# retrojetpacks/Gadget-Leicester

Measured on AMD Instinct MI355X. Metric: particle-steps/sec (gravity+SPH), higher is better.
Workload: dtype f64

## Files before the change

gadget-leicester_amd/csrc/ghip_gravity.hip:

```cpp
#include <cmath>

#include "ghip_prim.h"
#include "ghip_walk.h"

__global__ void k_grav_finish(int nt, const int *__restrict__ tgt, const int *__restrict__ perm,
                              int n, double G, double comoving_fac, const double *__restrict__ pos,
                              const double *__restrict__ gravpm, double *__restrict__ oacc,
                              double *__restrict__ oldacc)
{
  int ti = blockIdx.x * blockDim.x + threadIdx.x;
  if(ti >= nt)
    return;
  int i = perm[tgt[ti]];
  double a0 = oacc[i], a1 = oacc[(size_t) n + i], a2 = oacc[2 * (size_t) n + i];
  if(comoving_fac != 0)
    {
      a0 += comoving_fac * pos[i];
      a1 += comoving_fac * pos[(size_t) n + i];
      a2 += comoving_fac * pos[2 * (size_t) n + i];
    }
  double b0 = a0, b1 = a1, b2 = a2;
  if(gravpm)
    {
      b0 = a0 + gravpm[i] / G;
// ... 333 lines not shown
    sg.nsub = 1;
  sg.start = P<int>(t.seg_start) + t.seg_soff[table];
  sg.nanc = P<int>(t.seg_nanc) + t.seg_noff[table];
  sg.anc = P<int>(t.seg_anc) + (size_t) t.seg_noff[table] * GHIP_MAXANC;
  return sg.nsub;
}

static int walk_layout(const TreeDev &t, int nt, WalkSeg &sg, int *nbuckets, bool ewald)
{
  *nbuckets = (nt + 63) / 64;
  static int mid_min = -1;
  if(mid_min < 0)
    {
      mid_min = 3072;
      if(getenv("GHIP_WALK_MID_MIN"))
        mid_min = atoi(getenv("GHIP_WALK_MID_MIN"));
    }
  int table = ewald ? (*nbuckets >= mid_min ? 2 : 1) : (*nbuckets >= mid_min ? 1 : 0);
  return ghip_walk_layout(t, sg, table);
}

struct PartialBufs
{
  double *ax, *ay, *az;
  int *cost;
};

static int ensure_partials(ghip_ctx *ctx, int nwaves, int slot, PartialBufs &pb)
{
  size_t cnt = (size_t) nwaves * 64;
  DevBuf &bx = slot ? ctx->tax2 : ctx->tax, &by = slot ? ctx->tay2 : ctx->tay,
         &bz = slot ? ctx->taz2 : ctx->taz, &bc = slot ? ctx->tcost2 : ctx->tcost;
  GCHK(ghip_ensure(ctx, bx, cnt * 8));
  GCHK(ghip_ensure(ctx, by, cnt * 8));
  GCHK(ghip_ensure(ctx, bz, cnt * 8));
  GCHK(ghip_ensure(ctx, bc, cnt * 4));
  pb.ax = P<double>(bx);
  pb.ay = P<double>(by);
  pb.az = P<double>(bz);
  pb.cost = P<int>(bc);
  return GHIP_OK;
}

static int build_plan(ghip_ctx *ctx, int kind, int nb, int ns, WalkPlan &plan, int slot = 0,
                      hipStream_t on = nullptr)
{
  hipStream_t st = on ? on : ctx->stream;
  DevBuf &b_nsub = slot ? ctx->plan_nsub2 : ctx->plan_nsub, &b_woff = slot ? ctx->plan_woff2 : ctx->plan_woff,
         &b_wave = slot ? ctx->plan_wave2 : ctx->plan_wave;
  int sbase = (49152 + nb - 1) / nb;
  sbase = sbase < 8 ? 8 : (sbase > 64 ? 64 : sbase);
  if(sbase > ns)
    sbase = ns;
  if(getenv("GHIP_WALK_SUBS"))
    {
      int v = atoi(getenv("GHIP_WALK_SUBS"));
      if(v >= 1 && v <= ns)
        sbase = v;
    }
  const int maxwaves = (sbase + 2) * nb + 8;
  GCHK(ghip_ensure(ctx, b_nsub, (size_t) nb * 4));
  GCHK(ghip_ensure(ctx, b_woff, (size_t) (nb + 1) * 4));
  GCHK(ghip_ensure(ctx, b_wave, (size_t) maxwaves * 4));
  int cur = ctx->plan_cur[kind];
  bool prev_kept = ctx->plan_steps[kind][cur].p != nullptr;
  const size_t steps_bytes = ((size_t) nb + nb / 8 + 64) * 4;
  for(int k = 0; k < 2; k++)
    if(ctx->plan_steps[kind][k].cap < (size_t) nb * 4)
      {
        GCHK(ghip_ensure(ctx, ctx->plan_steps[kind][k], steps_bytes));
        if(k == cur)
          prev_kept = false;
      }
  const bool adaptive = !(getenv("GHIP_WALK_ADAPTIVE") && atoi(getenv("GHIP_WALK_ADAPTIVE")) == 0);
  const int pnb = ctx->plan_nb[kind];
  int tol = nb / 16 < 8 ? 8 : nb / 16;
  if(getenv("GHIP_PLAN_EXACT") && atoi(getenv("GHIP_PLAN_EXACT")))
    tol = ctx->plan_ns[kind] == ns ? 0 : -1;
  bool have_prev = adaptive && kind < 2 && pnb > 0 && (pnb > nb ? pnb - nb : nb - pnb) <= tol && prev_kept;
  int nprev = have_prev ? (pnb < nb ? pnb : nb) : 0;
  if(getenv("GHIP_PLAN_DEBUG") && kind < 2)
    {
      static int calls[2], used[2];
      calls[kind]++;
      used[kind] += have_prev;
      if(calls[kind] % 16 == 0)
        fprintf(stderr, "ghip plan kind %d: history used in %d of %d calls (nb %d, before %d)\n", kind,
                used[kind], calls[kind], nb, pnb);
    }
  unsigned int *prev = P<unsigned int>(ctx->plan_steps[kind][cur]);
  unsigned int *out = P<unsigned int>(ctx->plan_steps[kind][cur ^ 1]);
  k_plan_nsub<<<cdiv(nb, 256), 256, 0, st>>>(nb, ns, sbase, prev, nprev, P<int>(b_nsub));
  GCHK(ghip_scan(ctx, P<int>(b_nsub), P<int>(b_woff), nb, st, slot ? &ghip_prim_scratch(ctx, ctx->stream2) : nullptr));
  HIPCHK(hipMemsetAsync(b_wave.p, 0xff, (size_t) maxwaves * 4, st));
  k_plan_fill<<<cdiv(nb, 256), 256, 0, st>>>(nb, P<int>(b_nsub), P<int>(b_woff),
                                             maxwaves, P<int>(b_wave), out,
                                             ghip_errword(ctx, GHIP_ERRW_PLAN));
  HIPCHK(hipGetLastError());
  if(kind < 2)
    {
      ctx->plan_nb[kind] = nb;
      ctx->plan_ns[kind] = ns;
      ctx->plan_cur[kind] = cur ^ 1;
    }
  plan.nwaves = maxwaves;
  plan.wave_bucket = P<int>(b_wave);
  plan.woff = P<int>(b_woff);
  plan.nsub = P<int>(b_nsub);
  plan.steps_out = out;
  plan.started = nullptr;
  plan.started_at = 0;
  return GHIP_OK;
}

template <int MODE>
static void launch_walk(ghip_ctx *ctx, const TreeDev &t, const WalkSeg &sg, int nbuckets, int nt,
                        const int *tgt, const double *tx, const double *ty, const double *tz,
                        const double *tsoft, const double *toldacc, const GravK &k,
                        unsigned long long *counter, const WalkPlan &plan, const PartialBufs &pb,
                        hipStream_t stream)
{
  long long nthreads = (long long) plan.nwaves * 64;
  int bsize = 64;
  if(getenv("GHIP_WALK_BLOCK"))
    {
      int v = atoi(getenv("GHIP_WALK_BLOCK"));
      if(v == 64 || v == 128 || v == 256)
        bsize = v;
    }
  int blocks = cdiv(nthreads, bsize);
  blocks = (blocks + 7) & ~7;
  if(k.xcd_remap > 1)
    blocks = ((blocks + 8 * k.xcd_remap - 1) / (8 * k.xcd_remap)) * (8 * k.xcd_remap);
  WalkPlan pl = plan;
  if(pl.started)
    {
      static double frac = -1;
      if(frac < 0)
        frac = getenv("GHIP_HYDRO_TRIGGER_AT") ? atof(getenv("GHIP_HYDRO_TRIGGER_AT")) : 1.0;
      pl.started_at = (int) (frac * (blocks - 1));
      if(pl.started_at > blocks - 1 || pl.started_at < 0)
        pl.started_at = blocks - 1;
    }
  static int lds_env = -1;
  if(lds_env < 0)
    lds_env = getenv("GHIP_PAIR_NEWTON_LDS") ? atoi(getenv("GHIP_PAIR_NEWTON_LDS")) : 0;
  const int lds_n = lds_env > 0 ? lds_env : ctx->pair_lds;
  static int cap_min = -1;
  if(cap_min < 0)
    cap_min = getenv("GHIP_PAIR_CAP_MIN") ? atoi(getenv("GHIP_PAIR_CAP_MIN")) : 1536;
  static int lds_e = -1;
  if(lds_e < 0)
    lds_e = getenv("GHIP_PAIR_EWALD_LDS") ? atoi(getenv("GHIP_PAIR_EWALD_LDS")) : 0;
  const size_t dyn_lds =
    (MODE == GHIP_WALK_NEWTON && stream != ctx->stream && nbuckets >= cap_min)
      ? (size_t) lds_n
      : ((MODE == GHIP_WALK_EWALD && stream != ctx->stream && nbuckets >= cap_min) ? (size_t) lds_e : 0);
#define GHIP_LAUNCH_WALK(PER, UNEQ)                                                              \
  k_grav_walk<MODE, PER, UNEQ><<<blocks, bsize, dyn_lds, stream>>>(                                \
    t.nelem, P<WalkHot>(t.mq), P<WalkCold>(t.mq2), sg, nt, tgt, tx, ty, tz, tsoft, toldacc, k,     \
    P<float>(ctx->srtab), P<double>((UNEQ) && MODE == GHIP_WALK_EWALD ? ctx->ewbrick : ctx->ewtab),  \
    pb.ax, pb.ay, pb.az, pb.cost, getenv("GHIP_WALK_NOCOUNT") ? nullptr : counter,                  \
    P<unsigned long long>(ctx->rslots) + (counter - P<unsigned long long>(ctx->cslots)), pl)
  static int brick_env = -2;
  if(brick_env == -2)
    brick_env = getenv("GHIP_EW_BRICK") ? atoi(getenv("GHIP_EW_BRICK")) : -1;
  const bool brick = brick_env >= 0 ? brick_env != 0 : true;
  const bool uneq = (MODE == GHIP_WALK_EWALD) ? brick : (bool) k.unequal;
  if(k.periodic && uneq)
    GHIP_LAUNCH_WALK(true, true);
  else if(k.periodic)
    GHIP_LAUNCH_WALK(true, false);
  else if(uneq)
    GHIP_LAUNCH_WALK(false, true);
  else
    GHIP_LAUNCH_WALK(false, false);
#undef GHIP_LAUNCH_WALK
}

static void launch_walk_any(ghip_ctx *ctx, int walk, const TreeDev &t, const WalkSeg &sg,
                            int nbuckets, int nt, const int *tgt, const double *tx,
                            const double *ty, const double *tz, const double *tsoft,
                            const double *toldacc, const GravK &k, unsigned long long *counter,
                            const WalkPlan &plan, const PartialBufs &pb, hipStream_t stream)
{
  if(walk == GHIP_WALK_NEWTON)
    launch_walk<GHIP_WALK_NEWTON>(ctx, t, sg, nbuckets, nt, tgt, tx, ty, tz, tsoft, toldacc, k,
                                  counter, plan, pb, stream);
  else if(walk == GHIP_WALK_SHORTRANGE)
    launch_walk<GHIP_WALK_SHORTRANGE>(ctx, t, sg, nbuckets, nt, tgt, tx, ty, tz, tsoft, toldacc, k,
                                      counter, plan, pb, stream);
  else
    launch_walk<GHIP_WALK_EWALD>(ctx, t, sg, nbuckets, nt, tgt, tx, ty, tz, tsoft, toldacc, k,
                                 counter, plan, pb, stream);
}

static void shard_slice(const ghip_ctx *ctx, int nt, int *lo, int *cnt)
{
  int per;
  ghip_shard_range(nt, ctx->shard_n, ctx->shard_rank, lo, cnt, &per);
}

struct WalkJob
{
  int walk;
  GravK k;
  WalkSeg sg;
  WalkPlan plan;
  PartialBufs pb;
  int nbuckets;
  unsigned long long *counter;
};

static int prepare_job(ghip_ctx *ctx, const ghip_grav_params *p, int walk, int nt, int slot,
                       WalkJob &J, hipStream_t plan_on = nullptr)
{
  hipStream_t ps = plan_on ? plan_on : ctx->stream;
  J.walk = walk;
  GCHK(prepare_tables(ctx, p, walk, J.k));
  walk_layout(ctx->dyn_use ? ctx->dyn.tree : ctx->gt, nt, J.sg, &J.nbuckets, walk == GHIP_WALK_EWALD);
  GCHK(build_plan(ctx, walk == GHIP_WALK_EWALD ? 1 : 0, J.nbuckets, J.sg.ns, J.plan, slot, ps));
  GCHK(ensure_partials(ctx, J.plan.nwaves, slot, J.pb));
  J.counter = ghip_cslot(ctx, walk == GHIP_WALK_EWALD ? GHIP_CK_EWALD : GHIP_CK_NEWTON);
  HIPCHK(hipMemsetAsync(J.counter, 0, GHIP_CKIND_U64 * 8, ps));
  return GHIP_OK;
}

static int run_walk(ghip_ctx *ctx, const WalkJob &J, int nt, const int *tgt, hipStream_t st)
{
  int evi = (J.walk == GHIP_WALK_EWALD) ? 4 : 2;
  ctx->plan_writer[J.walk == GHIP_WALK_EWALD ? 1 : 0] = st;
  HIPCHK(hipEventRecord(ctx->evp[evi], st));
  launch_walk_any(ctx, J.walk, ctx->dyn_use ? ctx->dyn.tree : ctx->gt, J.sg, J.nbuckets, nt, tgt, P<double>(ctx->sx),
                  P<double>(ctx->sy), P<double>(ctx->sz), P<double>(ctx->ssoft),
                  P<double>(ctx->soldacc), J.k, J.counter, J.plan, J.pb, st);
  HIPCHK(hipGetLastError());
  HIPCHK(hipEventRecord(ctx->evp[evi + 1], st));
  return GHIP_OK;
}

static int combine_walk(ghip_ctx *ctx, const WalkJob &J, int nt, const int *tgt, hipStream_t st)
{
  k_combine_grav<<<cdiv(nt, 256), 256, 0, st>>>(
    nt, J.plan, tgt, P<int>(ctx->gt.perm), J.pb.ax, J.pb.ay, J.pb.az, J.pb.cost, ctx->n,
    P<double>(ctx->f[GHIP_F_GRAVACCEL]), P<int>(ctx->f[GHIP_F_GRAVCOST]),
    J.walk == GHIP_WALK_EWALD ? 1 : 0, J.k.debug_steps);
  HIPCHK(hipGetLastError());
  return GHIP_OK;
}

static const int pair_caps[GHIP_PAIR_NSET] = {GHIP_PAIR_LDS(6), GHIP_PAIR_LDS(5), GHIP_PAIR_LDS(4)};

static int pair_setting(int lds)
{
  int k = 0;
  for(int j = 1; j < GHIP_PAIR_NSET; j++)
    if(lds >= pair_caps[j])
      k = j;
  return k;
}

static int pair_balance(ghip_ctx *ctx)
{
  if(!ctx->pc_ev[3][3])
    {
      for(int i = 0; i < 4; i++)
        for(int j = 0; j < 4; j++)
          if(!ctx->pc_ev[i][j])
            HIPCHK(hipEventCreate(&ctx->pc_ev[i][j]));
      return GHIP_OK;
    }
  bool pending[GHIP_PAIR_NSET] = {};
  for(int i = 0; i < 4; i++)
    {
      if(ctx->pc_cap[i] == 0)
        continue;
      hipEvent_t *e = ctx->pc_ev[i];
      if(hipEventQuery(e[1]) != hipSuccess || hipEventQuery(e[3]) != hipSuccess)
        {
          (void) hipGetLastError();
          pending[pair_setting(ctx->pc_cap[i])] = true;
          continue;
        }
      float tn = 0, te = 0;
      if(hipEventElapsedTime(&tn, e[0], e[1]) == hipSuccess && hipEventElapsedTime(&te, e[2], e[3]) == hipSuccess)
        {
          const int k = pair_setting(ctx->pc_cap[i]);
          const float fe = ctx->pc_hyd[i] ? 1.1f : 1.0f;
          const float c = tn > fe * te ? tn : fe * te;
          ctx->pc_cost[k] = c;
          ctx->pc_age[k] = 0;
        }
      else
        (void) hipGetLastError();
      ctx->pc_cap[i] = 0;
    }
  for(int k = 0; k < GHIP_PAIR_NSET; k++)
    ctx->pc_age[k]++;
  const int cur = pair_setting(ctx->pair_lds);
  const float *cost = ctx->pc_cost;
  if(cost[cur] < 0)
    return GHIP_OK;
  int want = cur, probe = -1;
  for(int k = 0; k < GHIP_PAIR_NSET; k++)
    {
      if(k == cur || pending[k])
        continue;
      const bool close = cost[k] > 0 && cost[k] < 1.1f * cost[cur] && cost[cur] < 1.1f * cost[k];
      if(cost[k] < 0 || ctx->pc_age[k] > (close ? 16 : 64))
        {
// ... 293 lines not shown
```

gadget-leicester_amd/csrc/ghip_walk.h:

```cpp
#pragma once
#include "ghip_internal.h"
#include "ghip_count.h"

#ifndef GHIP_WALK_WAVES
#define GHIP_WALK_WAVES 8
#endif
#ifndef GHIP_WALK_OPT
#define GHIP_WALK_OPT 15
#endif


struct GravK
{
  double theta;
  double errtol;
  double boxsize, boxhalf;
  int periodic, unequal;
  int debug_steps;
  int xcd_remap;
  double rcut, rcut2, asmthfac;
  double fac_intp;
  double k1875;
};

// ... 52 lines not shown
template <class T>
__device__ __forceinline__ void d_touch(const T *__restrict__ base, int e, int &scratch)
{
  const unsigned int off = d_rec_off(e);
  asm volatile("s_load_dword %0, %1, %2" : "=s"(scratch) : "s"(base), "s"(off) : "memory");
}
template <class T>
__device__ __forceinline__ void d_load1_touch(const T *__restrict__ base, unsigned int off, v16i &R,
                                              int &s1, int &s2)
{
  asm volatile("s_load_dwordx16 %0, %3, %4\n\ts_waitcnt lgkmcnt(0)"
               : "=s"(R), "+s"(s1), "+s"(s2)
               : "s"(base), "s"(off)
               : "memory");
}
__device__ __forceinline__ void d_drain_touch(int &s1, int &s2)
{
  asm volatile("s_waitcnt lgkmcnt(0) ; drain-touches" : "+s"(s1), "+s"(s2) : : "memory");
}

__device__ __forceinline__ double d_rsqrt(double x)
{
  double y = __builtin_amdgcn_rsq(x);
  double t = x * y;
  double e = fma(-t, y, 1.0);
  double p = fma(0.375, e, 0.5);
  return fma(y * e, p, y);
}

__device__ __forceinline__ double d_mass_over_r3(double mass, double x, double k15 = 1.5,
                                                 double k1875 = 1.875)
{
  double y = __builtin_amdgcn_rsq(x);
  double y2 = y * y;
  double e = fma(-x, y2, 1.0);
  double p = fma(k1875, e, k15);
  double c = (mass * y) * y2;
  return fma(c * e, p, c);
}

struct SoftFac
{
  double fac, r;
};
static __device__ __attribute__((noinline, cold)) SoftFac d_grav_fac_inside(double mass, double r2,
                                                                            double h)
{
  SoftFac o;
  double r = sqrt(r2);
  o.r = r;
  double h_inv = 1.0 / h;
  double h3_inv = h_inv * h_inv * h_inv;
  double u = r * h_inv;
  if(u < 0.5)
    o.fac = mass * h3_inv * (10.666666666667 + u * u * (32.0 * u - 38.4));
  else
    o.fac = mass * h3_inv *
            (21.333333333333 - 48.0 * u + 38.4 * u * u - 10.666666666667 * u * u * u -
             0.066666666667 / (u * u * u));
  return o;
}

__device__ __forceinline__ double d_grav_fac(double mass, double r2, double h, double h2,
                                             double &r_out)
{
  if(r2 >= h2)
    {
      double rinv = d_rsqrt(r2);
      r_out = r2 * rinv;
      return mass * rinv * rinv * rinv;
    }
  const SoftFac s = d_grav_fac_inside(mass, r2, h);
  r_out = s.r;
  return s.fac;
}

template <bool BRICK>
__device__ __forceinline__ void d_ewald_interp(const double *__restrict__ tab, double fac_intp,
                                               double dx, double dy, double dz, double &fx,
                                               double &fy, double &fz)
{
  const int E1 = GHIP_EN + 1;
  const double sx = dx < 0 ? 1.0 : -1.0, sy = dy < 0 ? 1.0 : -1.0, sz = dz < 0 ? 1.0 : -1.0;
  dx = fabs(dx);
  dy = fabs(dy);
  dz = fabs(dz);
  double u = dx * fac_intp;
  int i = (int) u;
  if(i >= GHIP_EN)
    i = GHIP_EN - 1;
  u -= i;
  double v = dy * fac_intp;
  int j = (int) v;
  if(j >= GHIP_EN)
    j = GHIP_EN - 1;
  v -= j;
  double w = dz * fac_intp;
  int k = (int) w;
  if(k >= GHIP_EN)
    k = GHIP_EN - 1;
  w -= k;
  double f1 = (1 - u) * (1 - v) * (1 - w), f2 = (1 - u) * (1 - v) * (w);
  double f3 = (1 - u) * (v) * (1 - w), f4 = (1 - u) * (v) * (w);
  double f5 = (u) * (1 - v) * (1 - w), f6 = (u) * (1 - v) * (w);
  double f7 = (u) * (v) * (1 - w), f8 = (u) * (v) * (w);
  EwPair x00, x01, x10, x11, y00, y01, y10, y11, z00, z01, z10, z11;
  if(!BRICK)
    {
      const unsigned int ui = (unsigned int) i, uj = (unsigned int) j, uk = (unsigned int) k;
      const unsigned int R1 = E1 * 8u, R2 = E1 * E1 * 8u;
      const unsigned int ox = (ui * E1 + uj) * R1 + uk * 8u;
      const unsigned int oy = (uj * E1 + ui) * R1 + uk * 8u;
      const unsigned int oz = (uk * E1 + uj) * R1 + ui * 8u;
      const unsigned int ox2 = ox + R2, oy2 = oy + R2, oz2 = oz + R2;
      const char *tb = reinterpret_cast<const char *>(tab);
#define EW_LD(off, imm) d_ldpair(reinterpret_cast<const double *>(tb + (size_t) (off) + (imm)))
      x00 = EW_LD(ox, 0), x01 = EW_LD(ox, R1), x10 = EW_LD(ox2, 0), x11 = EW_LD(ox2, R1);
      y00 = EW_LD(oy, 0), y01 = EW_LD(oy, R1), y10 = EW_LD(oy2, 0), y11 = EW_LD(oy2, R1);
      z00 = EW_LD(oz, 0), z01 = EW_LD(oz, R1), z10 = EW_LD(oz2, 0), z11 = EW_LD(oz2, R1);
#undef EW_LD
    }
  else
    {
      const unsigned int SA = GHIP_EW_NB * GHIP_EW_NKB * 128, SB = GHIP_EW_NKB * 128;
      const unsigned int ai = (i >> 1) * SA + (i & 1) * 64, ai1 = ((i + 1) >> 1) * SA + ((i + 1) & 1) * 64;
      const unsigned int aj = (j >> 1) * SA + (j & 1) * 64, aj1 = ((j + 1) >> 1) * SA + ((j + 1) & 1) * 64;
      const unsigned int ak = (k >> 1) * SA + (k & 1) * 64, ak1 = ((k + 1) >> 1) * SA + ((k + 1) & 1) * 64;
      const unsigned int bi = (i >> 1) * SB + (i & 1) * 32, bi1 = ((i + 1) >> 1) * SB + ((i + 1) & 1) * 32;
      const unsigned int bj = (j >> 1) * SB + (j & 1) * 32, bj1 = ((j + 1) >> 1) * SB + ((j + 1) & 1) * 32;
      const unsigned int ck = ((((unsigned int) k * 43u) >> 7) * 13u + (unsigned int) k) * 8u;
      const unsigned int ci = ((((unsigned int) i * 43u) >> 7) * 13u + (unsigned int) i) * 8u;
      const char *tb = reinterpret_cast<const char *>(tab);
#define EW_LD(off) d_ldpair(reinterpret_cast<const double *>(tb + (off)))
      x00 = EW_LD(ai + bj + ck), x01 = EW_LD(ai + bj1 + ck), x10 = EW_LD(ai1 + bj + ck),
      x11 = EW_LD(ai1 + bj1 + ck);
      y00 = EW_LD(aj + bi + ck), y01 = EW_LD(aj + bi1 + ck), y10 = EW_LD(aj1 + bi + ck),
      y11 = EW_LD(aj1 + bi1 + ck);
      z00 = EW_LD(ak + bj + ci), z01 = EW_LD(ak + bj1 + ci), z10 = EW_LD(ak1 + bj + ci),
      z11 = EW_LD(ak1 + bj1 + ci);
#undef EW_LD
    }
  fx = sx * (x00.lo * f1 + x00.hi * f2 + x01.lo * f3 + x01.hi * f4 + x10.lo * f5 + x10.hi * f6 +
             x11.lo * f7 + x11.hi * f8);
  fy = sy * (y00.lo * f1 + y00.hi * f2 + y10.lo * f3 + y10.hi * f4 + y01.lo * f5 + y01.hi * f6 +
             y11.lo * f7 + y11.hi * f8);
  fz = sz * (z00.lo * f1 + z10.lo * f2 + z01.lo * f3 + z11.lo * f4 + z00.hi * f5 + z10.hi * f6 +
             z01.hi * f7 + z11.hi * f8);
}

struct WalkLane
{
  double pos_x, pos_y, pos_z, h_i, aold;
  double h2;
  double k15;
  double acc_x, acc_y, acc_z;
  int nint;
};

__device__ __forceinline__ double d_nearest1(double x, double boxsize, double boxhalf)
{
  return (fabs(x) > boxhalf) ? x - copysign(boxsize, x) : x;
}

__device__ __forceinline__ double d_nearest1_masked(double x, double boxsize, double boxhalf)
{
  if(fabs(x) > boxhalf)
    {
      x -= copysign(boxsize, x);
      asm volatile("" : "+v"(x));
    }
  return x;
}

typedef unsigned long long lmask;
#define D_BAL(cond) __builtin_amdgcn_ballot_w64(cond)
#define D_LANE(mask) __builtin_amdgcn_inverse_ballot_w64(mask)

__device__ __forceinline__ void d_skip_to(int &my_skip, int skip)
{
  asm volatile("v_max_i32 %0, %1, %0" : "+v"(my_skip) : "s"(skip));
}

template <int MODE, bool PERIODIC, bool UNEQUAL, bool OWNED, bool REL>
__device__ __forceinline__ int d_walk_element(int e, const v16i &H,
                                              const WalkCold *__restrict__ cold, const GravK &p,
                                              const float *__restrict__ srtab,
                                              const double *__restrict__ ewtab, WalkLane &W,
                                              int &my_skip)
{
  const double ex = d_f64(H, 0), ey = d_f64(H, 1), ez = d_f64(H, 2), mass = d_f64(H, 3);
  const double mlen2 = d_f64(H, 4), len2 = d_f64(H, 5);
  const int skip = d_lo32(H, 6), pidx = d_hi32(H, 6);
  const double aux = d_f64(H, 7);
  const lmask act = D_BAL(e >= my_skip);
  int next;

  double dx = ex - W.pos_x, dy = ey - W.pos_y, dz = ez - W.pos_z;
  double r2;
  if((GHIP_WALK_OPT & 1) && (MODE == GHIP_WALK_EWALD || PERIODIC))
    {
      r2 = dx * dx + dy * dy + dz * dz;
      if(D_BAL(r2 >= p.boxhalf * p.boxhalf) != 0)
        {
          if(D_LANE(D_BAL(fabs(dx) > p.boxhalf)))
            {
              dx -= copysign(p.boxsize, dx);
              asm volatile("" : "+v"(dx));
            }
          if(D_LANE(D_BAL(fabs(dy) > p.boxhalf)))
            {
              dy -= copysign(p.boxsize, dy);
              asm volatile("" : "+v"(dy));
            }
          if(D_LANE(D_BAL(fabs(dz) > p.boxhalf)))
            {
              dz -= copysign(p.boxsize, dz);
              asm volatile("" : "+v"(dz));
            }
          r2 = dx * dx + dy * dy + dz * dz;
        }
    }
  else if(MODE == GHIP_WALK_EWALD || PERIODIC)
    {
      const lmask wx = D_BAL(fabs(dx) > p.boxhalf), wy = D_BAL(fabs(dy) > p.boxhalf),
                  wz = D_BAL(fabs(dz) > p.boxhalf);
      if((wx | wy | wz) != 0)
        {
          if(D_LANE(wx))
            {
              dx -= copysign(p.boxsize, dx);
              asm volatile("" : "+v"(dx));
            }
          if(D_LANE(wy))
            {
              dy -= copysign(p.boxsize, dy);
              asm volatile("" : "+v"(dy));
            }
          if(D_LANE(wz))
            {
              dz -= copysign(p.boxsize, dz);
              asm volatile("" : "+v"(dz));
            }
        }
      r2 = dx * dx + dy * dy + dz * dz;
    }
  else
    r2 = dx * dx + dy * dy + dz * dz;
  double h = W.h_i, h2 = W.h2;
  lmask interact;

  if(pidx >= 0)
    {
      next = e + 1;
      interact = act;
      if(MODE != GHIP_WALK_EWALD && UNEQUAL)
        {
          if(h < aux)
            {
              h = aux;
              h2 = h * h;
            }
        }
    }
  else
    {
      lmask gt, rel;
      if(REL)
        {
          gt = D_BAL(mlen2 > r2 * r2 * W.aold);
          rel = ~0ull;
        }
      else
        {
          gt = D_BAL(len2 > r2 * p.theta * p.theta);
          rel = 0ull;
        }
      lmask open = act & gt;
      lmask far = act & ~gt & rel;
      lmask drop = 0;
      const double len2x4 = __hiloint2double(d_hi32(H, 5) + 0x00200000, d_lo32(H, 5));
      const lmask boxcand = far & D_BAL(r2 < len2x4);
      lmask cutcand = 0;
      if(MODE == GHIP_WALK_SHORTRANGE)
        cutcand = act & D_BAL(r2 > p.rcut2);
      lmask need_cold = boxcand;
      if(MODE == GHIP_WALK_SHORTRANGE)
        need_cold |= cutcand;
      if(MODE == GHIP_WALK_EWALD)
        need_cold |= open;
      if(need_cold != 0)
        {
          v16i C;
          d_load1(cold, e, C);
          const double cx = d_f64(C, 0), cy = d_f64(C, 1), cz = d_f64(C, 2), len = d_f64(C, 3);
          const double len06 = d_f64(C, 4);
          const double c0 = cx - W.pos_x, c1 = cy - W.pos_y, c2 = cz - W.pos_z;
          if(MODE == GHIP_WALK_SHORTRANGE)
            {
              if(cutcand != 0)
                {
                  double eff = p.rcut + 0.5 * len;
                  double d0 = c0, d1 = c1, d2 = c2;
                  if(PERIODIC)
                    {
                      d0 = d_nearest1(d0, p.boxsize, p.boxhalf);
                      d1 = d_nearest1(d1, p.boxsize, p.boxhalf);
                      d2 = d_nearest1(d2, p.boxsize, p.boxhalf);
                    }
                  drop = cutcand &
                         (D_BAL(fabs(d0) > eff) | D_BAL(fabs(d1) > eff) | D_BAL(fabs(d2) > eff));
                }
              open &= ~drop;
              far &= ~drop;
            }
          if(far != 0)
            open |= far & D_BAL(fabs(c0) < len06) & D_BAL(fabs(c1) < len06) &
                    D_BAL(fabs(c2) < len06);
          if(MODE == GHIP_WALK_EWALD)
            {
              if(open != 0 && !(len > 0.20 * p.boxsize))
                {
                  double u0 = d_nearest1(c0, p.boxsize, p.boxhalf);
                  double u1 = d_nearest1(c1, p.boxsize, p.boxhalf);
                  double u2 = d_nearest1(c2, p.boxsize, p.boxhalf);
                  double lim = 0.5 * (p.boxsize - len);
                  open &= D_BAL(fabs(u0) > lim) | D_BAL(fabs(u1) > lim) | D_BAL(fabs(u2) > lim);
                }
            }
        }
      if(MODE != GHIP_WALK_EWALD && UNEQUAL)
        {
          const double ms = fabs(aux);
          const lmask up = act & ~drop & ~open & D_BAL(h < ms);
          if(up != 0)
            {
              if(D_LANE(up))
                {
                  h = ms;
                  h2 = ms * ms;
                }
              if(aux < 0)
                open |= up & D_BAL(r2 < ms * ms);
            }
        }
      interact = act & ~drop & ~open;
      if(!((GHIP_WALK_OPT & 4) && OWNED && MODE == GHIP_WALK_NEWTON) || (interact & D_BAL(r2 < h2)) != 0)
        if(D_LANE(interact | drop))
          d_skip_to(my_skip, skip);
      next = skip;
      if(open != 0)
        {
          next = e + 1;
          if(skip == next)
            {
              int *w = *(int *volatile *) &d_walk_errw;
              if(w)
                *(volatile int *) w = 1;
            }
        }
    }

  if(OWNED && MODE == GHIP_WALK_NEWTON && (interact & D_BAL(r2 < h2)) == 0)
    {
      const int counted = pidx & 1;
      const int sk = skip;
      if(D_LANE(interact))
        {
          const double fac = (GHIP_WALK_OPT & 8) ? d_mass_over_r3(mass, r2, W.k15, p.k1875)
                                                 : d_mass_over_r3(mass, r2);
          W.acc_x += dx * fac;
          W.acc_y += dy * fac;
          W.acc_z += dz * fac;
          if(GHIP_WALK_OPT & 2)
            W.nint += counted;
          else
            W.nint += (mass > 0) ? 1 : 0;
          if(GHIP_WALK_OPT & 4)
            d_skip_to(my_skip, sk);
        }
      return next;
    }
  if(OWNED && D_LANE(interact))
    {
      if(MODE == GHIP_WALK_EWALD)
        {
          double fx, fy, fz;
          d_ewald_interp<UNEQUAL>(ewtab, p.fac_intp, dx, dy, dz, fx, fy, fz);
          W.acc_x += mass * fx;
          W.acc_y += mass * fy;
          W.acc_z += mass * fz;
          W.nint++;
        }
      else
        {
          double r;
          double fac = d_grav_fac(mass, r2, h, h2, r);
          if(MODE == GHIP_WALK_SHORTRANGE)
            {
              int tabindex = (int) (p.asmthfac * r);
              if(tabindex < GHIP_NTAB)
                {
                  fac *= srtab[tabindex];
                  W.acc_x += dx * fac;
                  W.acc_y += dy * fac;
                  W.acc_z += dz * fac;
                  W.nint++;
                }
            }
          else
            {
              W.acc_x += dx * fac;
              W.acc_y += dy * fac;
              W.acc_z += dz * fac;
              if(mass > 0)
                W.nint++;
            }
        }
    }
  return next;
}

struct WalkPlan
{
  int nwaves;
  const int *__restrict__ wave_bucket;
  const int *__restrict__ woff;
  const int *__restrict__ nsub;
  unsigned int *__restrict__ steps_out;
  unsigned int *started;
  int started_at;
};

struct SegCursor
{
  int kseg;
  int e, s1;
};

template <int MODE, bool PERIODIC, bool UNEQUAL, bool REL>
__device__ __forceinline__ bool d_enter_segment(SegCursor &c, int stride, const WalkSeg &sg,
                                                const WalkHot *__restrict__ hot,
                                                const WalkCold *__restrict__ cold, const GravK &p,
                                                const float *__restrict__ srtab,
                                                const double *__restrict__ ewtab, bool valid,
                                                WalkLane &W, int &my_skip, unsigned int &steps)
{
  while(c.kseg < sg.ns)
    {
      const int s0 = __builtin_amdgcn_readfirstlane(sg.start[c.kseg]);
      c.s1 = __builtin_amdgcn_readfirstlane(sg.start[c.kseg + 1]);
      my_skip = valid ? 0 : 0x7fffffff;
      const int na = __builtin_amdgcn_readfirstlane(sg.nanc[c.kseg]);
      for(int a = 0; a < na; a++)
        {
          int ea = __builtin_amdgcn_readfirstlane(sg.anc[c.kseg * GHIP_MAXANC + a]);
          v16i H;
          d_load1(hot, ea, H);
          d_walk_element<MODE, PERIODIC, UNEQUAL, false, REL>(ea, H, cold, p, srtab, ewtab, W, my_skip);
          steps++;
        }
      int first = d_wave_min_i32(my_skip);
      c.e = __builtin_amdgcn_readfirstlane(first > s0 ? first : s0);
      if(c.e < c.s1)
        return true;
      c.kseg += stride;
    }
  return false;
}

template <int MODE, bool PERIODIC, bool UNEQUAL, bool REL>
__device__ __forceinline__ void d_walk_run(const WalkSeg &sg, int sub, const WalkHot *__restrict__ hot,
                                           const WalkCold *__restrict__ cold, const GravK &p,
                                           const float *__restrict__ srtab,
                                           const double *__restrict__ ewtab, bool valid, WalkLane &W,
                                           unsigned int &steps)
{
  if(MODE != GHIP_WALK_EWALD)
    {
      SegCursor A;
      int skipA = 0;
      A.kseg = sub;
      const int stride = sg.nsub;
      bool liveA = d_enter_segment<MODE, PERIODIC, UNEQUAL, REL>(A, stride, sg, hot, cold, p, srtab,
                                                            ewtab, valid, W, skipA, steps);
      int t1 = 0, t2 = 0;
      while(liveA)
        {
          v16i HA;
          const unsigned int offA = d_rec_off(A.e);
          d_load1_touch(hot, offA, HA, t1, t2);
          d_touch_next(hot, offA, t1);
          d_touch(hot, d_lo32(HA, 6), t2);
          steps++;
          A.e = __builtin_amdgcn_readfirstlane(
            d_walk_element<MODE, PERIODIC, UNEQUAL, true, REL>(A.e, HA, cold, p, srtab, ewtab, W, skipA));
          if(__builtin_expect(A.e >= A.s1, 0))
            {
              d_drain_touch(t1, t2);
              A.kseg += stride;
              liveA = d_enter_segment<MODE, PERIODIC, UNEQUAL, REL>(A, stride, sg, hot, cold, p, srtab,
                                                               ewtab, valid, W, skipA, steps);
            }
        }
      d_drain_touch(t1, t2);
    }
  else
    {
      SegCursor A, B;
      int skipA = 0, skipB = 0;
      A.kseg = sub;
      B.kseg = sub + sg.nsub;
      const int stride = 2 * sg.nsub;
      bool liveA = d_enter_segment<MODE, PERIODIC, UNEQUAL, REL>(A, stride, sg, hot, cold, p, srtab, ewtab, valid,
                                                   W, skipA, steps);
      bool liveB = d_enter_segment<MODE, PERIODIC, UNEQUAL, REL>(B, stride, sg, hot, cold, p, srtab, ewtab, valid,
                                                   W, skipB, steps);
      while(liveA && liveB)
        {
          v16i HA, HB;
          d_load2(hot, A.e, HA, B.e, HB);
          steps += 2;
          A.e = __builtin_amdgcn_readfirstlane(
            d_walk_element<MODE, PERIODIC, UNEQUAL, true, REL>(A.e, HA, cold, p, srtab, ewtab, W, skipA));
          B.e = __builtin_amdgcn_readfirstlane(
            d_walk_element<MODE, PERIODIC, UNEQUAL, true, REL>(B.e, HB, cold, p, srtab, ewtab, W, skipB));
          if(A.e >= A.s1)
            {
              A.kseg += stride;
              liveA = d_enter_segment<MODE, PERIODIC, UNEQUAL, REL>(A, stride, sg, hot, cold, p, srtab, ewtab,
                                                      valid, W, skipA, steps);
            }
          if(B.e >= B.s1)
            {
              B.kseg += stride;
              liveB = d_enter_segment<MODE, PERIODIC, UNEQUAL, REL>(B, stride, sg, hot, cold, p, srtab, ewtab,
                                                      valid, W, skipB, steps);
            }
        }
      if(liveB)
        {
          A = B;
          skipA = skipB;
          liveA = true;
        }
      while(liveA)
        {
          v16i HA;
          d_load1(hot, A.e, HA);
          steps++;
          A.e = __builtin_amdgcn_readfirstlane(
            d_walk_element<MODE, PERIODIC, UNEQUAL, true, REL>(A.e, HA, cold, p, srtab, ewtab, W, skipA));
          if(A.e >= A.s1)
            {
              A.kseg += stride;
              liveA = d_enter_segment<MODE, PERIODIC, UNEQUAL, REL>(A, stride, sg, hot, cold, p, srtab, ewtab,
                                                      valid, W, skipA, steps);
            }
        }
    }

}

template <int MODE, bool PERIODIC, bool UNEQUAL>
__global__ void __launch_bounds__(GHIP_BLOCK) __attribute__((amdgpu_waves_per_eu(MODE == GHIP_WALK_EWALD ? 4 : GHIP_WALK_WAVES, 8)))
k_grav_walk(int nelem, const WalkHot *__restrict__ hot, const WalkCold *__restrict__ cold,
            WalkSeg sg, int nt, const int *__restrict__ tgt, const double *__restrict__ tx,
            const double *__restrict__ ty, const double *__restrict__ tz,
            const double *__restrict__ tsoft, const double *__restrict__ toldacc, GravK p,
            const float *__restrict__ srtab, const double *__restrict__ ewtab,
            double *__restrict__ pax, double *__restrict__ pay, double *__restrict__ paz,
            int *__restrict__ pcost, unsigned long long *__restrict__ counter,
            unsigned long long *__restrict__ acc, WalkPlan plan)
{
  const int lane = threadIdx.x & 63;
  if(plan.started && blockIdx.x == plan.started_at && threadIdx.x == 0)
    __hip_atomic_store(plan.started, 1u, __ATOMIC_RELEASE, __HIP_MEMORY_SCOPE_SYSTEM);
  const int per_xcd = gridDim.x >> 3;
  int lblock = blockIdx.x;
  if(p.xcd_remap == 1)
    lblock = (blockIdx.x & 7) * per_xcd + (blockIdx.x >> 3);
  else if(p.xcd_remap > 1)
    {
      const int j = blockIdx.x >> 3, x = blockIdx.x & 7, G = p.xcd_remap;
      lblock = ((j / G) * 8 + x) * G + (j % G);
    }
  const int wave = __builtin_amdgcn_readfirstlane((lblock * (int) blockDim.x + threadIdx.x) >> 6);
  if(wave >= plan.nwaves)
    return;
  const int bucket = __builtin_amdgcn_readfirstlane(plan.wave_bucket[wave]);
  if(bucket < 0 || bucket * 64 >= nt)
    return;
  const int sub = wave - __builtin_amdgcn_readfirstlane(plan.woff[bucket]);
  sg.nsub = __builtin_amdgcn_readfirstlane(plan.nsub[bucket]);
  const int ti = bucket * 64 + lane;
  const bool valid = ti < nt;
  const int s = valid ? (tgt ? tgt[ti] : ti) : 0;

  WalkLane W;
  W.pos_x = W.pos_y = W.pos_z = 0;
  W.h_i = 1;
  W.aold = 0;
  W.h2 = 1;
  if(valid)
    {
      W.pos_x = tx[s];
      W.pos_y = ty[s];
      W.pos_z = tz[s];
      W.h_i = tsoft[s];
      W.aold = p.errtol * toldacc[s];
      W.h2 = W.h_i * W.h_i;
    }
  W.acc_x = W.acc_y = W.acc_z = 0;
  W.nint = 0;
  W.k15 = 1.5;
  asm volatile("" : "+v"(W.k15));
  unsigned int steps = 0;

  if(p.theta == 0)
    d_walk_run<MODE, PERIODIC, UNEQUAL, true>(sg, sub, hot, cold, p, srtab, ewtab, valid, W, steps);
  else
    d_walk_run<MODE, PERIODIC, UNEQUAL, false>(sg, sub, hot, cold, p, srtab, ewtab, valid, W, steps);

  if(valid)
    {
      const size_t o = (size_t) wave * 64 + lane;
      pax[o] = W.acc_x;
      pay[o] = W.acc_y;
      paz[o] = W.acc_z;
      pcost[o] = p.debug_steps ? (int) steps : W.nint;
    }
  unsigned long long tot = d_wave_sum_u64((unsigned long long) W.nint);
  if(lane == 0 && tot && counter)
    {
      d_count(counter, 0, tot);
      d_count(acc, 0, tot);
    }
  if(lane == 0)
    {
      if(counter)
        {
          d_count(counter, 1, (unsigned long long) steps);
          d_count(acc, 1, (unsigned long long) steps);
        }
      atomicAdd(plan.steps_out + bucket, steps);
    }
}

__global__ void k_plan_nsub(int nb, int ns, int sbase, const unsigned int *__restrict__ steps_prev,
                            int nprev, int *__restrict__ nsub)
{
  __shared__ unsigned long long part[4];
  unsigned long long tot = 0;
  if(nprev > 0)
    {
      for(int k = threadIdx.x; k < nprev; k += blockDim.x)
        tot += steps_prev[k];
      for(int o = 32; o > 0; o >>= 1)
        tot += __shfl_xor(tot, o);
      if((threadIdx.x & 63) == 0)
        part[threadIdx.x >> 6] = tot;
      __syncthreads();
      tot = part[0] + part[1] + part[2] + part[3];
    }
  int b = blockIdx.x * blockDim.x + threadIdx.x;
  if(b >= nb)
    return;
  int s = ns < sbase ? ns : sbase;
  if(b < nprev && tot > 0)
    {
      double mean = (double) tot / (double) nprev;
      s = (int) ((double) sbase * (double) steps_prev[b] / mean) + 1;
      s = s < 2 ? 2 : s;
      s = s > 64 ? 64 : s;
      if(s > ns)
        s = ns;
    }
  nsub[b] = s < 1 ? 1 : s;
}

__global__ void k_plan_fill(int nb, const int *__restrict__ nsub, const int *__restrict__ woff,
                            int maxwaves, int *__restrict__ wave_bucket,
                            unsigned int *__restrict__ steps_out, int *__restrict__ errword)
{
  int b = blockIdx.x * blockDim.x + threadIdx.x;
  if(b >= nb)
    return;
  int o = woff[b], s = nsub[b];
  if(o + s > maxwaves)
    *(volatile int *) errword = 1;
  for(int q = 0; q < s; q++)
    if(o + q < maxwaves)
      wave_bucket[o + q] = b;
  steps_out[b] = 0;
}

struct SegTables
{
  int ntab;
  int ns[3], soff[3], noff[3];
};

__global__ void k_build_segments(const TreeSizes *__restrict__ ts, const int4 *__restrict__ lk,
                                 SegTables T, int *__restrict__ start, int *__restrict__ nanc,
                                 int *__restrict__ anc)
{
  const int nelem = ts->nelem;
  int g = blockIdx.x * blockDim.x + threadIdx.x;
  int j = 0;
  while(j < T.ntab && g > T.ns[j])
    {
      g -= T.ns[j] + 1;
      j++;
    }
  if(j >= T.ntab)
    return;
  const int ns = T.ns[j], k = g;
  start += T.soff[j];
  nanc += T.noff[j];
  anc += (size_t) T.noff[j] * GHIP_MAXANC;
  long long chunk = ((long long) nelem + ns - 1) / ns;
  long long s0l = (long long) k * chunk;
  int s0 = (int) (s0l > nelem ? nelem : s0l);
  if(k == ns)
    s0 = nelem;
  start[k] = s0;
  if(k == ns)
    return;
  int na = 0, e = 0;
  while(e < s0)
    {
      int4 q = lk[e];
      if(!LK_IS_PARTICLE(q) && q.x > s0)
        {
          if(na < GHIP_MAXANC)
            anc[k * GHIP_MAXANC + na] = e;
          na++;
          e = e + 1;
        }
      else
        e = q.x;
    }
  nanc[k] = na < GHIP_MAXANC ? na : GHIP_MAXANC;
}

__global__ void k_combine_grav(int nt, WalkPlan plan, const int *__restrict__ tgt,
                               const int *__restrict__ perm, const double *__restrict__ pax,
                               const double *__restrict__ pay, const double *__restrict__ paz,
                               const int *__restrict__ pcost, int n, double *__restrict__ oacc,
                               int *__restrict__ ocost, int accumulate, int debug_max)
{
  int ti = blockIdx.x * blockDim.x + threadIdx.x;
  if(ti >= nt)
    return;
  const int bucket = ti >> 6, lane = ti & 63;
  const int w0 = plan.woff[bucket];
  int nsub = plan.nsub[bucket];
  if(w0 + nsub > plan.nwaves)
    nsub = plan.nwaves > w0 ? plan.nwaves - w0 : 0;
  double a0 = 0, a1 = 0, a2 = 0;
  int c = 0;
  for(int s = 0; s < nsub; s++)
    {
      size_t o = (size_t) (w0 + s) * 64 + lane;
      a0 += pax[o];
      a1 += pay[o];
      a2 += paz[o];
      c = debug_max ? (pcost[o] > c ? pcost[o] : c) : c + pcost[o];
    }
  int i = perm ? perm[tgt[ti]] : ti;
  if(accumulate)
    {
      oacc[i] += a0;
      oacc[(size_t) n + i] += a1;
      oacc[2 * (size_t) n + i] += a2;
      ocost[i] += c;
    }
  else
    {
      oacc[i] = a0;
      oacc[(size_t) n + i] = a1;
      oacc[2 * (size_t) n + i] = a2;
      ocost[i] = c;
    }
}

__global__ void k_combine_pair(int nt, WalkPlan pn, WalkPlan pe, const int *__restrict__ tgt,
                               const int *__restrict__ perm, const double *__restrict__ nax,
                               const double *__restrict__ nay, const double *__restrict__ naz,
                               const int *__restrict__ ncost, const double *__restrict__ eax,
                               const double *__restrict__ eay, const double *__restrict__ eaz,
                               const int *__restrict__ ecost, int n, double *__restrict__ oacc,
                               int *__restrict__ ocost)
{
  int ti = blockIdx.x * blockDim.x + threadIdx.x;
  if(ti >= nt)
    return;
  const int bucket = ti >> 6, lane = ti & 63;
  double a0 = 0, a1 = 0, a2 = 0, b0 = 0, b1 = 0, b2 = 0;
  int c = 0, d = 0;
// ... 75 lines not shown
```

Measured before the change: 85.51 million.

## Cut walk kernel VGPR use: softening in LDS, wave-max h2 test, DPP reductions

Result: slower. 82.63 million (-3.4%).

```diff
diff --git a/gadget-leicester_amd/csrc/ghip_gravity.hip b/gadget-leicester_amd/csrc/ghip_gravity.hip
--- a/gadget-leicester_amd/csrc/ghip_gravity.hip
+++ b/gadget-leicester_amd/csrc/ghip_gravity.hip
@@ -509,10 +509,12 @@
   static int lds_e = -1;
   if(lds_e < 0)
     lds_e = getenv("GHIP_PAIR_EWALD_LDS") ? atoi(getenv("GHIP_PAIR_EWALD_LDS")) : 0;
-  const size_t dyn_lds =
+  size_t dyn_lds =
     (MODE == GHIP_WALK_NEWTON && stream != ctx->stream && nbuckets >= cap_min)
       ? (size_t) lds_n
       : ((MODE == GHIP_WALK_EWALD && stream != ctx->stream && nbuckets >= cap_min) ? (size_t) lds_e : 0);
+  if(MODE == GHIP_WALK_NEWTON && !k.unequal && dyn_lds < (size_t) bsize * sizeof(double))
+    dyn_lds = (size_t) bsize * sizeof(double);
 #define GHIP_LAUNCH_WALK(PER, UNEQ)                                                              \
   k_grav_walk<MODE, PER, UNEQ><<<blocks, bsize, dyn_lds, stream>>>(                                \
     t.nelem, P<WalkHot>(t.mq), P<WalkCold>(t.mq2), sg, nt, tgt, tx, ty, tz, tsoft, toldacc, k,     \
diff --git a/gadget-leicester_amd/csrc/ghip_walk.h b/gadget-leicester_amd/csrc/ghip_walk.h
--- a/gadget-leicester_amd/csrc/ghip_walk.h
+++ b/gadget-leicester_amd/csrc/ghip_walk.h
@@ -228,10 +228,28 @@
 {
   double pos_x, pos_y, pos_z, h_i, aold;
   double h2;
-  double k15;
   double acc_x, acc_y, acc_z;
   int nint;
+  int h2max_hi;
+  int slot0;
+  int bh2_hi;
+  double k15, k1875;
 };
+
+extern __shared__ double d_walk_lds[];
+
+template <int MODE, bool UNEQUAL>
+__device__ __forceinline__ constexpr bool d_soft_wave()
+{
+  return MODE == GHIP_WALK_NEWTON && !UNEQUAL;
+}
+
+__device__ __forceinline__ int d_lane_here()
+{
+  int l;
+  asm volatile("v_mbcnt_lo_u32_b32 %0, -1, 0\n\tv_mbcnt_hi_u32_b32 %0, -1, %0" : "=&v"(l));
+  return l;
+}
 
 __device__ __forceinline__ double d_nearest1(double x, double boxsize, double boxhalf)
 {
@@ -252,9 +270,53 @@
 #define D_BAL(cond) __builtin_amdgcn_ballot_w64(cond)
 #define D_LANE(mask) __builtin_amdgcn_inverse_ballot_w64(mask)
 
+__device__ __forceinline__ double d_shift_box(double x, double boxhalf)
+{
+  int shi, slo;
+  asm("v_lshrrev_b32 %0, 31, %2\n\tv_lshl_or_b32 %0, %0, 31, %3\n\tv_mov_b32 %1, %4"
+      : "=&v"(shi), "=&v"(slo)
+      : "v"(__double2hiint(x)), "s"(__double2hiint(boxhalf)), "s"(__double2loint(boxhalf)));
+  const double sh = __hiloint2double(shi, slo);
+  x = fma(-2.0, sh, x);
+  asm volatile("" : "+v"(x));
+  return x;
+}
+
 __device__ __forceinline__ void d_skip_to(int &my_skip, int skip)
 {
   asm volatile("v_max_i32 %0, %1, %0" : "+v"(my_skip) : "s"(skip));
+}
+
+#define D_DPP(ident, v, ctrl, rows) __builtin_amdgcn_update_dpp((int) (ident), (int) (v), ctrl, rows, 0xf, false)
+#define D_DPP_STEPS(STEP) STEP(0x111, 0xf) STEP(0x112, 0xf) STEP(0x114, 0xf) STEP(0x118, 0xf) STEP(0x142, 0xa) STEP(0x143, 0xc)
+__device__ __forceinline__ int d_walk_min_i32(int v)
+{
+#define STEP(ctrl, rows)                              \
+  {                                                   \
+    const int o = D_DPP(0x7fffffff, v, ctrl, rows);   \
+    v = o < v ? o : v;                                \
+  }
+  D_DPP_STEPS(STEP)
+#undef STEP
+  return __builtin_amdgcn_readlane(v, 63);
+}
+__device__ __forceinline__ unsigned int d_walk_sum_u32(unsigned int v)
+{
+#define STEP(ctrl, rows) v += (unsigned int) D_DPP(0, v, ctrl, rows);
+  D_DPP_STEPS(STEP)
+#undef STEP
+  return (unsigned int) __builtin_amdgcn_readlane((int) v, 63);
+}
+__device__ __forceinline__ unsigned int d_walk_max_u32(unsigned int v)
+{
+#define STEP(ctrl, rows)                                       \
+  {                                                            \
+    const unsigned int o = (unsigned int) D_DPP(0, v, ctrl, rows); \
+    v = o > v ? o : v;                                         \
+  }
+  D_DPP_STEPS(STEP)
+#undef STEP
+  return (unsigned int) __builtin_amdgcn_readlane((int) v, 63);
 }
 
 template <int MODE, bool PERIODIC, bool UNEQUAL, bool OWNED, bool REL>
@@ -276,22 +338,19 @@
   if((GHIP_WALK_OPT & 1) && (MODE == GHIP_WALK_EWALD || PERIODIC))
     {
       r2 = dx * dx + dy * dy + dz * dz;
-      if(D_BAL(r2 >= p.boxhalf * p.boxhalf) != 0)
+      if(D_BAL((unsigned int) __double2hiint(r2) >= (unsigned int) W.bh2_hi) != 0)
         {
           if(D_LANE(D_BAL(fabs(dx) > p.boxhalf)))
             {
-              dx -= copysign(p.boxsize, dx);
-              asm volatile("" : "+v"(dx));
+              dx = d_shift_box(dx, p.boxhalf);
             }
           if(D_LANE(D_BAL(fabs(dy) > p.boxhalf)))
             {
-              dy -= copysign(p.boxsize, dy);
-              asm volatile("" : "+v"(dy));
+              dy = d_shift_box(dy, p.boxhalf);
             }
           if(D_LANE(D_BAL(fabs(dz) > p.boxhalf)))
             {
-              dz -= copysign(p.boxsize, dz);
-              asm volatile("" : "+v"(dz));
+              dz = d_shift_box(dz, p.boxhalf);
             }
           r2 = dx * dx + dy * dy + dz * dz;
         }
@@ -304,25 +363,24 @@
         {
           if(D_LANE(wx))
             {
-              dx -= copysign(p.boxsize, dx);
-              asm volatile("" : "+v"(dx));
+              dx = d_shift_box(dx, p.boxhalf);
             }
           if(D_LANE(wy))
             {
-              dy -= copysign(p.boxsize, dy);
-              asm volatile("" : "+v"(dy));
+              dy = d_shift_box(dy, p.boxhalf);
             }
           if(D_LANE(wz))
             {
-              dz -= copysign(p.boxsize, dz);
-              asm volatile("" : "+v"(dz));
+              dz = d_shift_box(dz, p.boxhalf);
             }
         }
       r2 = dx * dx + dy * dy + dz * dz;
     }
   else
     r2 = dx * dx + dy * dy + dz * dz;
-  double h = W.h_i, h2 = W.h2;
+  constexpr bool SOFTW = d_soft_wave<MODE, UNEQUAL>();
+  double h = SOFTW ? 0.0 : W.h_i, h2 = SOFTW ? 0.0 : W.h2;
+#define D_SOFT_LANES() (SOFTW ? D_BAL((unsigned int) __double2hiint(r2) <= (unsigned int) W.h2max_hi) : D_BAL(r2 < h2))
   lmask interact;
 
   if(pidx >= 0)
@@ -420,7 +478,7 @@
             }
         }
       interact = act & ~drop & ~open;
-      if(!((GHIP_WALK_OPT & 4) && OWNED && MODE == GHIP_WALK_NEWTON) || (interact & D_BAL(r2 < h2)) != 0)
+      if(!((GHIP_WALK_OPT & 4) && OWNED && MODE == GHIP_WALK_NEWTON) || (interact & D_SOFT_LANES()) != 0)
         if(D_LANE(interact | drop))
           d_skip_to(my_skip, skip);
       next = skip;
@@ -431,18 +489,22 @@
             {
               int *w = *(int *volatile *) &d_walk_errw;
               if(w)
-                *(volatile int *) w = 1;
-            }
-        }
-    }
-
-  if(OWNED && MODE == GHIP_WALK_NEWTON && (interact & D_BAL(r2 < h2)) == 0)
+                {
+                  int one = 1;
+                  asm volatile("" : "+v"(one));
+                  *(volatile int *) w = one;
+                }
+            }
+        }
+    }
+
+  if(OWNED && MODE == GHIP_WALK_NEWTON && __builtin_expect((interact & D_SOFT_LANES()) == 0, 1))
     {
       const int counted = pidx & 1;
       const int sk = skip;
       if(D_LANE(interact))
         {
-          const double fac = (GHIP_WALK_OPT & 8) ? d_mass_over_r3(mass, r2, W.k15, p.k1875)
+          const double fac = (GHIP_WALK_OPT & 8) ? d_mass_over_r3(mass, r2, W.k15, SOFTW ? W.k1875 : p.k1875)
                                                  : d_mass_over_r3(mass, r2);
           W.acc_x += dx * fac;
           W.acc_y += dy * fac;
@@ -469,8 +531,24 @@
         }
       else
         {
-          double r;
-          double fac = d_grav_fac(mass, r2, h, h2, r);
+          double r, fac;
+          if(SOFTW)
+            {
+              h = d_walk_lds[W.slot0 + d_lane_here()];
+              h2 = h * h;
+              const lmask inside = D_BAL(r2 < h2);
+              fac = r2;
+              if(D_LANE(inside))
+                fac = d_grav_fac_inside(mass, fac, h).fac;
+              asm volatile("" : "+v"(fac));
+              if(!D_LANE(inside))
+                {
+                  const double rinv = d_rsqrt(fac);
+                  fac = mass * rinv * rinv * rinv;
+                }
+            }
+          else
+            fac = d_grav_fac(mass, r2, h, h2, r);
           if(MODE == GHIP_WALK_SHORTRANGE)
             {
               int tabindex = (int) (p.asmthfac * r);
@@ -494,6 +572,7 @@
         }
     }
   return next;
+#undef D_SOFT_LANES
 }
 
 struct WalkPlan
@@ -535,7 +614,7 @@
           d_walk_element<MODE, PERIODIC, UNEQUAL, false, REL>(ea, H, cold, p, srtab, ewtab, W, my_skip);
           steps++;
         }
-      int first = d_wave_min_i32(my_skip);
+      int first = d_walk_min_i32(my_skip);
       c.e = __builtin_amdgcn_readfirstlane(first > s0 ? first : s0);
       if(c.e < c.s1)
         return true;
@@ -637,16 +716,19 @@
 
 }
 
+#define GHIP_WALK_PARAMS \
+  int nelem, const WalkHot *__restrict__ hot, const WalkCold *__restrict__ cold, \
+  WalkSeg sg, int nt, const int *__restrict__ tgt, const double *__restrict__ tx, \
+  const double *__restrict__ ty, const double *__restrict__ tz, \
+  const double *__restrict__ tsoft, const double *__restrict__ toldacc, GravK p, \
+  const float *__restrict__ srtab, const double *__restrict__ ewtab, \
+  double *__restrict__ pax, double *__restrict__ pay, double *__restrict__ paz, \
+  int *__restrict__ pcost, unsigned long long *__restrict__ counter, \
+  unsigned long long *__restrict__ acc, WalkPlan plan
+#define GHIP_WALK_ARGS \
+  nelem, hot, cold, sg, nt, tgt, tx, ty, tz, tsoft, toldacc, p, srtab, ewtab, pax, pay, paz, pcost, counter, acc, plan
 template <int MODE, bool PERIODIC, bool UNEQUAL>
-__global__ void __launch_bounds__(GHIP_BLOCK) __attribute__((amdgpu_waves_per_eu(MODE == GHIP_WALK_EWALD ? 4 : GHIP_WALK_WAVES, 8)))
-k_grav_walk(int nelem, const WalkHot *__restrict__ hot, const WalkCold *__restrict__ cold,
-            WalkSeg sg, int nt, const int *__restrict__ tgt, const double *__restrict__ tx,
-            const double *__restrict__ ty, const double *__restrict__ tz,
-            const double *__restrict__ tsoft, const double *__restrict__ toldacc, GravK p,
-            const float *__restrict__ srtab, const double *__restrict__ ewtab,
-            double *__restrict__ pax, double *__restrict__ pay, double *__restrict__ paz,
-            int *__restrict__ pcost, unsigned long long *__restrict__ counter,
-            unsigned long long *__restrict__ acc, WalkPlan plan)
+__device__ __forceinline__ void d_grav_walk(GHIP_WALK_PARAMS)
 {
   const int lane = threadIdx.x & 63;
   if(plan.started && blockIdx.x == plan.started_at && threadIdx.x == 0)
@@ -670,14 +752,17 @@
   sg.nsub = __builtin_amdgcn_readfirstlane(plan.nsub[bucket]);
   const int ti = bucket * 64 + lane;
   const bool valid = ti < nt;
-  const int s = valid ? (tgt ? tgt[ti] : ti) : 0;
+  constexpr bool MIRROR = d_soft_wave<MODE, UNEQUAL>();
+  const bool walks = MIRROR || valid;
+  const int tw = (MIRROR && !valid) ? bucket * 64 : ti;
+  const int s = walks ? (tgt ? tgt[tw] : tw) : 0;
 
   WalkLane W;
   W.pos_x = W.pos_y = W.pos_z = 0;
   W.h_i = 1;
   W.aold = 0;
   W.h2 = 1;
-  if(valid)
+  if(walks)
     {
       W.pos_x = tx[s];
       W.pos_y = ty[s];
@@ -686,32 +771,49 @@
       W.aold = p.errtol * toldacc[s];
       W.h2 = W.h_i * W.h_i;
     }
+  W.h2max_hi = 0;
+  W.slot0 = 0;
+  if(d_soft_wave<MODE, UNEQUAL>())
+  {
+    W.h2max_hi = (int) d_walk_max_u32((unsigned int) __double2hiint(W.h2));
+    W.slot0 = __builtin_amdgcn_readfirstlane((int) threadIdx.x) & ~63;
+    d_walk_lds[threadIdx.x] = W.h_i;
+  }
   W.acc_x = W.acc_y = W.acc_z = 0;
   W.nint = 0;
   W.k15 = 1.5;
   asm volatile("" : "+v"(W.k15));
+  W.k1875 = 1.875;
+  if(d_soft_wave<MODE, UNEQUAL>())
+    asm volatile("" : "+v"(W.k1875));
+  W.bh2_hi = __builtin_amdgcn_readfirstlane(__double2hiint(p.boxhalf * p.boxhalf));
+  asm volatile("" : "+s"(W.bh2_hi));
   unsigned int steps = 0;
 
   if(p.theta == 0)
-    d_walk_run<MODE, PERIODIC, UNEQUAL, true>(sg, sub, hot, cold, p, srtab, ewtab, valid, W, steps);
+    d_walk_run<MODE, PERIODIC, UNEQUAL, true>(sg, sub, hot, cold, p, srtab, ewtab, walks, W, steps);
   else
-    d_walk_run<MODE, PERIODIC, UNEQUAL, false>(sg, sub, hot, cold, p, srtab, ewtab, valid, W, steps);
-
+    d_walk_run<MODE, PERIODIC, UNEQUAL, false>(sg, sub, hot, cold, p, srtab, ewtab, walks, W, steps);
+
+  if(MIRROR && !valid)
+    W.nint = 0;
+  const int lane_out = d_lane_here();
   if(valid)
     {
-      const size_t o = (size_t) wave * 64 + lane;
+      const size_t o = (size_t) wave * 64 + lane_out;
       pax[o] = W.acc_x;
       pay[o] = W.acc_y;
       paz[o] = W.acc_z;
       pcost[o] = p.debug_steps ? (int) steps : W.nint;
     }
-  unsigned long long tot = d_wave_sum_u64((unsigned long long) W.nint);
-  if(lane == 0 && tot && counter)
+  unsigned long long tot = (unsigned long long) d_walk_sum_u32((unsigned int) W.nint & 0xffffu) +
+                           ((unsigned long long) d_walk_sum_u32((unsigned int) W.nint >> 16) << 16);
+  if(lane_out == 0 && tot && counter)
     {
       d_count(counter, 0, tot);
       d_count(acc, 0, tot);
     }
-  if(lane == 0)
+  if(lane_out == 0)
     {
       if(counter)
         {
@@ -721,6 +823,24 @@
       atomicAdd(plan.steps_out + bucket, steps);
     }
 }
+
+template <int MODE, bool PERIODIC, bool UNEQUAL>
+__global__ void __launch_bounds__(GHIP_BLOCK) __attribute__((amdgpu_waves_per_eu(MODE == GHIP_WALK_EWALD ? 4 : GHIP_WALK_WAVES, 8)))
+k_grav_walk(GHIP_WALK_PARAMS)
+{
+  d_grav_walk<MODE, PERIODIC, UNEQUAL>(GHIP_WALK_ARGS);
+}
+#define GHIP_WALK_48(PERIODIC)                                                                              \
+  template <>                                                                                               \
+  __global__ void __launch_bounds__(GHIP_BLOCK)                                                             \
+    __attribute__((amdgpu_waves_per_eu(GHIP_WALK_WAVES, 8), amdgpu_num_vgpr(24)))                           \
+    k_grav_walk<GHIP_WALK_NEWTON, PERIODIC, false>(GHIP_WALK_PARAMS)                                        \
+  {                                                                                                         \
+    d_grav_walk<GHIP_WALK_NEWTON, PERIODIC, false>(GHIP_WALK_ARGS);                                         \
+  }
+GHIP_WALK_48(true)
+GHIP_WALK_48(false)
+#undef GHIP_WALK_48
 
 __global__ void k_plan_nsub(int nb, int ns, int sbase, const unsigned int *__restrict__ steps_prev,
                             int nprev, int *__restrict__ nsub)
```
